# g8a9/multi-modal-emotion

Hardware: AMD Instinct MI355X
Metric: utterances/sec fwd+bwd (+clip_grad_norm_+AdamW inside the timed step), TAV (BERT+Wav2Vec2+VideoMAE) b=32, 1/2/4/8 MI355X (higher is better)
Workload: dtype bf16; 1 GPU; tav_nn.py TAV preset B (bert 12 L + wav2vec2 12 L / 768 + videomae 12 L / 768 on 16 frames + fusion 12 L), global batch 32 = 32 per GPU x 1, text 128 tok, audio 80000 samples, video 16x3x224x224 (104 fusion / 1464 encoder tokens), 547.0 GFLOP forward per utterance; global_batch=32, per_gpu_batch=32, parallelism=dp1, weights=random init (seeded), no checkpoints offline, launch=hipGraph replay

## Files before the change

include/tavhip.h:

```cpp
#ifndef TAVHIP_H
#define TAVHIP_H
#include <stdint.h>

#ifdef __cplusplus
extern "C" {
#endif

enum { TAV_F32 = 0, TAV_BF16 = 1, TAV_FP8 = 2 ,
       TAV_U8 = 3 ,
       TAV_I16 = 4  };
enum {
    TAV_ERR_NULL = -1,
    TAV_ERR_SHAPE = -2,
    TAV_ERR_DTYPE = -3,
    TAV_ERR_ALIGN = -4,
    TAV_ERR_NO_RCCL = -5
};

int tav_version(void);
const char* tav_error_string(int code);

typedef struct tav_gemm_nt_args {
    const void* A; const void* B; void* C;
    void* C_pre;
    const float* bias;
    const void* gelu_in;
    const float* resid;
    int64_t M, N, K;
    int64_t lda, ldb, ldc, ld_pre, ld_gelu_in, ld_resid;
    int32_t nzb, nzg;
    int64_t a_zb, a_zg, b_zb, b_zg, c_zb, c_zg, bias_zg;
    int32_t in_dtype, out_dtype;
    int32_t act;
    int32_t accumulate;
    float alpha;
    const float* a_dequant;
    const float* b_dequant;
    int64_t gelu_zb;
    int32_t tile_m_hint;
} tav_gemm_nt_args;
int tav_gemm_nt(const tav_gemm_nt_args* args, void* stream);
int tav_gemm_nt_schedule(const tav_gemm_nt_args* args, int32_t* tile, int32_t* rows_first, int32_t* tile_rest);

typedef struct tav_gemm_tn_args {
    const void* A; const void* B;
    float* slabs;
    float* out;
    float* dbias;
    float* bias_partials;
    int64_t N1, N2;
    int64_t lda, ldb;
    int64_t rows_per_batch, nbatch;
    int64_t a_zb, b_zb;
    int32_t chunk_rows, nsplit;
    int32_t perm_inner, perm_outer;
    int32_t dtype;
    int32_t accumulate;
    float scale;
} tav_gemm_tn_args;
int tav_gemm_tn_splits(int64_t n1, int64_t n2, int64_t rows_per_batch, int64_t nbatch, int32_t* chunk_rows, int32_t* nsplit);
int tav_gemm_tn(const tav_gemm_tn_args* args, void* stream);

typedef struct tav_gemm_tn_problem {
    const void* A; const void* B;
    float* out;
    float* dbias;
    int64_t N1, N2, lda, ldb;
} tav_gemm_tn_problem;
int tav_gemm_tn_grouped(const tav_gemm_tn_problem* problems, int32_t nproblems, int64_t rows, int32_t dtype, void* stream);
int64_t tav_gemm_tn_grouped_ws_bytes(const tav_gemm_tn_problem* problems, int32_t nproblems, int64_t rows, int32_t dtype, int32_t flags);
int tav_gemm_tn_grouped_ws(const tav_gemm_tn_problem* problems, int32_t nproblems, int64_t rows, int32_t dtype, void* workspace,
                           int64_t workspace_bytes, int32_t flags, void* stream);

int tav_fp8_amax_partials(int64_t rows, int64_t cols);
int tav_fp8_amax(const void* x, int32_t dtype, int64_t rows, int64_t cols, int64_t ld, float* partials, float* scales, void* stream);
int tav_fp8_quantize(const void* x, int32_t dtype, int64_t rows, int64_t cols, int64_t ld, const float* scales, void* q, int64_t ld_q, void* qt,
                     int64_t ld_qt, int64_t rows_pad, void* stream);
int tav_fp8_quantize_delayed(const void* x, int32_t dtype, int64_t rows, int64_t cols, int64_t ld, float* state, void* q, int64_t ld_q, void* qt,
                             int64_t ld_qt, int64_t rows_pad, void* stream);
int tav_fp8_roll_states(float* states, int64_t n, void* stream);
int tav_splitk_reduce(const float* slabs, float* out, int32_t nsplit, int64_t n_elems, int32_t accumulate, void* stream);

int tav_colsum(const void* x, int32_t dtype, int64_t M, int64_t N, int64_t ld, float* partials, int32_t nparts, float* out,
               int32_t accumulate, void* stream);

typedef struct tav_attn_args {
    const void* q; const void* k; const void* v;
    void* o;
    const float* key_mask;
    float* lse;
    float* corr;
    void* o_soft;
    const void* dout; void* dq; void* dk; void* dv;
    float* delta;
    int64_t B, S, nheads;
    int64_t ld_q, ld_k, ld_v, ld_o, ld_do, ld_dq, ld_dk, ld_dv;
    int32_t dtype, mask_mode;
    float scale;
    int32_t q_prescaled;
} tav_attn_args;
int tav_attn_fwd(const tav_attn_args* args, void* stream);
int tav_attn_bwd(const tav_attn_args* args, void* stream);
int tav_attn_fwd_len(const tav_attn_args* args, const int32_t* seq_lens, void* stream);
int tav_attn_bwd_len(const tav_attn_args* args, const int32_t* seq_lens, void* stream);
int tav_attn_probs(const tav_attn_args* args, float* probs, const float* head_scale, int64_t hs_bstride, void* stream);
int tav_head_scale(const void* a, const void* b, void* out, int32_t dtype, const float* head_scale, int64_t hs_bstride, float c0, int64_t B, int64_t S,
                   int64_t nheads, int64_t lda, int64_t ldb, int64_t ldo, void* stream);

typedef struct tav_ln_args {
    const void* x; int32_t x_dtype;
    const float* gamma; const float* beta;
    float* y_f32; void* y_lp; int32_t lp_dtype;
    float* mean; float* rstd;
    const void* dy; int32_t dy_dtype;
    const float* dx_add;
    float* dx_f32; void* dx_lp;
    float* dgamma; float* dbeta; float* partials; int32_t accumulate_params;
    int64_t rows, W;
    int64_t ld_x, ld_y, ld_dy, ld_dx;
    float eps;
    int32_t act;
    int32_t defer_param_reduce;
} tav_ln_args;
// ... 172 lines not shown
```

multi-modal-emotion_amd/csrc/gemm_plan.h:

```cpp
#pragma once
#include <stdint.h>
#include <algorithm>
#include "../../include/tavhip.h"

namespace tav {
namespace plan {

inline int elem_size(int dtype) { return dtype == TAV_FP8 ? 1 : (dtype == TAV_BF16 ? 2 : 4); }

inline int nt_validate(const tav_gemm_nt_args* a, bool need_ptrs) {
    if (!a || (need_ptrs && (!a->A || !a->B || !a->C))) return TAV_ERR_NULL;
    if (a->M <= 0 || a->N <= 0 || a->K <= 0) return TAV_ERR_SHAPE;
    const int es = elem_size(a->in_dtype);
    if (a->in_dtype != TAV_BF16 && a->in_dtype != TAV_F32 && a->in_dtype != TAV_FP8) return TAV_ERR_DTYPE;
    if (a->in_dtype == TAV_F32 && a->out_dtype != TAV_F32) return TAV_ERR_DTYPE;
    if (a->out_dtype != TAV_F32 && a->out_dtype != TAV_BF16) return TAV_ERR_DTYPE;
    if ((a->K * es) % 128 != 0) return TAV_ERR_SHAPE;
    if ((a->M * a->lda + a->K) * es >= (1ll << 32) || (a->N * a->ldb + a->K) * es >= (1ll << 32)) return TAV_ERR_SHAPE;
    if (a->N % 4 != 0) return TAV_ERR_SHAPE;
    {
        const int64_t ldmax = std::max(std::max(a->ldc, a->C_pre ? a->ld_pre : 0), std::max(a->gelu_in ? a->ld_gelu_in : 0, a->resid ? a->ld_resid : 0));
        if (ldmax < 0 || 256 * ldmax + a->N >= (1ll << 30)) return TAV_ERR_SHAPE;
    }
    const int pk = 16 / es;
    if (a->lda % pk || a->ldb % pk || a->ldc % 4) return TAV_ERR_ALIGN;
    if (a->a_zb % pk || a->a_zg % pk || a->b_zb % pk || a->b_zg % pk || a->c_zb % 4 || a->c_zg % 4 || a->gelu_zb % 4) return TAV_ERR_ALIGN;
    return 0;
}

inline int nt_small_tile(int M, int N, int nz) {
    const int tiles_n = (N + 127) / 128;
    int tm = 4;
    double best = 1e30;
    for (int c = 4; c >= 2; --c) {
        const long tiles = (long)((M + 32 * c - 1) / (32 * c)) * tiles_n * nz;
        const double cost = (double)((tiles + 255) / 256) * (c + 0.8);
        if (cost < best - 1e-9) { best = cost; tm = c; }
    }
    return tm;
}
inline double nt_small_us(int M, int N, double nk, int nz, int tm, int epi) {
    static const double slots[5] = {0, 0, 768, 512, 512}, tk[5] = {0, 0, 0.56, 0.72, 0.85}, fix[5] = {0, 0, 3.6, 4.0, 4.4};
    const long t = (long)((M + 32 * tm - 1) / (32 * tm)) * ((N + 127) / 128) * nz;
    const double e = ((epi & 1) ? 2.0 + 0.2 * nk : 0.0) + ((epi & 2) ? 2.0 : 0.0) + ((epi & 4) ? 2.0 : 0.0) + ((epi & 8) ? 1.0 : 0.0) + ((epi & 16) ? 2.5 : 0.0);
    const double kt = (nk <= 36.0 ? nk : 36.0 + 1.6 * (nk - 36.0)) * tk[tm];
    return (double)((long)((t + slots[tm] - 1) / slots[tm])) * (kt + fix[tm] + e * tm / 4.0);
}
inline double nt_big_round_us(double nk, int epi) {
    const double kt = nk * 1.45;
    return kt + 6.5 + ((epi & 1) ? 9.0 : 0.0) + ((epi & 2) ? 4.0 : 0.0) + ((epi & 4) ? 3.0 : 0.0) + ((epi & 8) ? 4.7 : 0.0) + ((epi & 16) ? 6.7 : 0.0);
}
inline int nt_pick_tile(int M, int N, int K, int nz, bool bf16_in, int epi, int* rows_big = nullptr, int* tm_rest = nullptr) {
    int tm = nt_small_tile(M, N, nz);
    if (rows_big) *rows_big = M;
    if (bf16_in && M >= 256 && N >= 256) {
        const double nk = (double)K / 64.0;
        const long tn_big = (N + 255) / 256;
        const long t_big = (long)((M + 255) / 256) * tn_big * nz;
        const double us_small = nt_small_us(M, N, nk, nz, tm, epi);
        const double big_round = nt_big_round_us(nk, epi);
        const double us_big = (double)((t_big + 255) / 256) * big_round;
        double us_best = us_small;
        if (us_big < 0.98 * us_small) { tm = 16; us_best = us_big; }
        const long full = t_big / 256;
        if (rows_big && nz == 1 && full >= 1 && t_big % 256 != 0) {
            const long m_tiles = full * 256 / tn_big;
            const int rows_a = (int)(m_tiles * 256), m_rest = M - rows_a;
            if (m_tiles >= 1 && m_rest > 0) {
                const int tr = nt_small_tile(m_rest, N, 1);
                const double us_split = (double)((m_tiles * tn_big + 255) / 256) * big_round + nt_small_us(m_rest, N, nk, 1, tr, epi) + 2.0;
                if (us_split < 0.93 * us_best) { tm = 16; *rows_big = rows_a; *tm_rest = tr; }
            }
        }
    }
    return tm;
}
inline void nt_plan(const tav_gemm_nt_args* a, int* tm_out, int* rows_big, int* tm_rest) {
    const int es = elem_size(a->in_dtype);
    const int nz = (int)((a->nzb > 0 ? a->nzb : 1) * (a->nzg > 0 ? a->nzg : 1));
    int tm = a->tile_m_hint & 31;
    const bool may_split = tm == 0 && a->in_dtype == TAV_BF16 && nz == 1;
    *rows_big = (int)a->M; *tm_rest = 4;
    if (a->in_dtype == TAV_F32 && (tm == 8 || tm == 16)) tm = 4;
    if (tm != 8 && tm != 16 && (tm < 2 || tm > 4))
        tm = nt_pick_tile((int)a->M, (int)a->N, (int)(a->K * es / 2), nz, a->in_dtype != TAV_F32,
                          ((a->resid || a->accumulate) ? 1 : 0) | (a->out_dtype == TAV_F32 ? 2 : 0) | ((a->act & 3) ? 4 : 0) | (a->gelu_in ? 8 : 0) | (a->C_pre ? 16 : 0),
                          may_split ? rows_big : nullptr, tm_rest);
    if (a->in_dtype == TAV_FP8 && tm != 16) tm = 4;
    *tm_out = tm;
}

enum { EPI_GEN = 0, EPI_PLAIN = 1, EPI_RESID = 2, EPI_GELU_D = 3, EPI_MUL_D = 4 };

#define TAV_NT_TILES(X, IN, OUT, NST, EPI) X(IN, OUT, 4, NST, 4, 4, EPI) X(IN, OUT, 3, NST, 4, 4, EPI) X(IN, OUT, 2, NST, 4, 4, EPI)
#define TAV_NT_FLAVOUR(X, IN, OUT, EPI) X(IN, OUT, 4, 2, 8, 8, EPI) TAV_NT_TILES(X, IN, OUT, 4, EPI) TAV_NT_TILES(X, IN, OUT, 2, EPI)
#define TAV_NT_FLAVOUR3(X, IN, OUT, EPI) \
    X(IN, OUT, 4, 2, 8, 8, EPI) X(IN, OUT, 4, 3, 8, 4, GEN) TAV_NT_TILES(X, IN, OUT, 4, EPI) TAV_NT_TILES(X, IN, OUT, 3, GEN) TAV_NT_TILES(X, IN, OUT, 2, EPI)
#define TAV_NT_KERNELS(X)                                                                                                        \
                                  \
    X(FP8, BF16, 4, 2, 8, 8, PLAIN) X(FP8, BF16, 4, 2, 8, 8, GELU_D) X(FP8, BF16, 4, 2, 8, 8, MUL_D) X(FP8, BF16, 4, 2, 8, 8, GEN) \
    X(FP8, F32, 4, 2, 8, 8, PLAIN) X(FP8, F32, 4, 2, 8, 8, RESID) X(FP8, F32, 4, 2, 8, 8, GEN)                                    \
    X(FP8, BF16, 4, 2, 4, 4, GEN) X(FP8, F32, 4, 2, 4, 4, GEN)                                                                    \
    TAV_NT_FLAVOUR3(X, BF16, BF16, PLAIN) TAV_NT_FLAVOUR(X, BF16, BF16, GELU_D) TAV_NT_FLAVOUR(X, BF16, BF16, MUL_D) TAV_NT_FLAVOUR(X, BF16, BF16, GEN) \
    TAV_NT_FLAVOUR3(X, BF16, F32, PLAIN) TAV_NT_FLAVOUR(X, BF16, F32, RESID) TAV_NT_FLAVOUR(X, BF16, F32, GEN)                    \
                                                                               \
    X(F32, F32, 4, 2, 4, 4, GEN) X(F32, F32, 3, 2, 4, 4, GEN) X(F32, F32, 2, 2, 4, 4, GEN)

struct NtKey {
    int8_t in, out, tm, nst, nw, tnw, epi;
};
constexpr bool operator==(const NtKey& a, const NtKey& b) {
    return a.in == b.in && a.out == b.out && a.tm == b.tm && a.nst == b.nst && a.nw == b.nw && a.tnw == b.tnw && a.epi == b.epi;
}
#define TAV_NT_KEY(IN, OUT, TM, NST, NW, TNW, EPI) {TAV_##IN, TAV_##OUT, TM, NST, NW, TNW, EPI_##EPI},
constexpr NtKey nt_keys[] = {TAV_NT_KERNELS(TAV_NT_KEY)};
#undef TAV_NT_KEY
constexpr int nt_num_keys = (int)(sizeof(nt_keys) / sizeof(nt_keys[0]));
inline int nt_key_index(const NtKey& k) {
    for (int i = 0; i < nt_num_keys; ++i)
        if (nt_keys[i] == k) return i;
    return -1;
}

struct NtLaunch {
    NtKey key;
    int tiles_m, tiles_n;
    unsigned grid_x, grid_y, block;
    size_t lds;
};
inline NtLaunch nt_launch(const tav_gemm_nt_args* a, int M, int tm) {
    const int in = a->in_dtype, out = a->out_dtype;
    const int nzb = a->nzb > 0 ? a->nzb : 1, nzg = a->nzg > 0 ? a->nzg : 1;
    const int bm = tm >= 8 ? 256 : 32 * tm, bn = tm == 16 ? 256 : 128;
    NtLaunch L;
    L.tiles_m = (M + bm - 1) / bm;
    L.tiles_n = ((int)a->N + bn - 1) / bn;
    const long wgs = (long)L.tiles_m * L.tiles_n * nzb * nzg;
    int nst = (a->tile_m_hint >> 5) & 7;
    if (tm == 8) nst = 3;
    else if (tm == 16) nst = 2;
    else if (nst < 2 || nst > 4) nst = (wgs <= 256 && in == TAV_BF16) ? 4 : 2;
    if (in != TAV_BF16) nst = 2;
    L.grid_x = (unsigned)(L.tiles_m * L.tiles_n); L.grid_y = (unsigned)(nzb * nzg); L.block = tm >= 8 ? 512 : 256;
    L.lds = (tm == 16 && in == TAV_BF16) ? (size_t)160 * 1024 : (size_t)nst * (bm + bn) * 128;
    const bool side = a->resid || a->C_pre || a->gelu_in || a->accumulate;
    int epi = EPI_GEN;
    if (!side && a->act == 0) epi = EPI_PLAIN;
    else if (a->resid && !a->C_pre && !a->gelu_in && !a->accumulate && a->act == 0 && out == TAV_F32) epi = EPI_RESID;
    else if (a->C_pre && (a->act & 3) == 3 && !a->resid && !a->gelu_in && !a->accumulate && out == TAV_BF16) epi = EPI_GELU_D;
    else if (a->gelu_in && (a->act & 4) && !(a->act & 3) && !a->resid && !a->C_pre && !a->accumulate && out == TAV_BF16) epi = EPI_MUL_D;
    if (nst == 3 || in == TAV_F32 || (in == TAV_FP8 && tm != 16)) epi = EPI_GEN;
    L.key = NtKey{(int8_t)in, (int8_t)out, (int8_t)(tm >= 8 ? 4 : tm), (int8_t)nst, (int8_t)(tm >= 8 ? 8 : 4), (int8_t)(tm == 16 ? 8 : 4), (int8_t)epi};
    return L;
}

struct NtSplit {
    int M_rest;
    long a_bytes, c_bytes, pre_bytes, gelu_bytes, resid_elems;
};
inline NtSplit nt_split(const tav_gemm_nt_args* a, int rows_big) {
    const long r = rows_big, es = elem_size(a->in_dtype), oes = elem_size(a->out_dtype);
    return NtSplit{(int)a->M - rows_big, r * a->lda * es, r * a->ldc * oes, r * a->ld_pre * oes, r * a->ld_gelu_in * es, r * a->ld_resid};
}

constexpr int TN_PROBLEMS_MAX = 4;

inline int tn_validate_problem(const void* A, const void* B, const void* out, int64_t N1, int64_t N2, int64_t lda, int64_t ldb, int64_t a_zb,
                               int64_t b_zb, int64_t rows_per_batch, int64_t nbatch, int dtype) {
    if (!A || !B || !out) return TAV_ERR_NULL;
    if (N1 <= 0 || N2 <= 0 || rows_per_batch <= 0 || nbatch <= 0) return TAV_ERR_SHAPE;
    if (dtype != TAV_BF16 && dtype != TAV_F32) return TAV_ERR_DTYPE;
    const int es = elem_size(dtype), pk = 16 / es;
    if (N1 % pk || N2 % pk || N2 % 4) return TAV_ERR_SHAPE;
    if (lda % pk || ldb % pk || a_zb % pk || b_zb % pk) return TAV_ERR_ALIGN;
    if ((rows_per_batch + 64) * (lda > ldb ? lda : ldb) * es >= (1ll << 32)) return TAV_ERR_SHAPE;
    return 0;
}
inline int tn_validate_group(const tav_gemm_tn_problem* probs, int nprob, int64_t rows, int dtype) {
    for (int k = 0; k < nprob; ++k) {
        const tav_gemm_tn_problem& a = probs[k];
        const int rc = tn_validate_problem(a.A, a.B, a.out, a.N1, a.N2, a.lda, a.ldb, 0, 0, rows, 1, dtype);
        if (rc != 0) return rc;
    }
    return 0;
}

constexpr double TN_SPLIT_PENALTY = 0.06;
inline void tn_splits(int64_t n1, int64_t n2, int64_t rows_per_batch, int64_t nbatch, int32_t* chunk_rows, int32_t* nsplit) {
    const long tiles = ((n1 + 127) / 128) * ((n2 + 127) / 128);
    const long SLOTS = 512;
    long best_cpb = 1, best_cr = ((rows_per_batch + 63) / 64) * 64; double best_score = -1.0;
    const long max_cpb = (rows_per_batch + 255) / 256 > 0 ? (rows_per_batch + 255) / 256 : 1;
    for (long cpb = 1; cpb <= max_cpb && cpb <= 64; ++cpb) {
        long cr = (rows_per_batch + cpb - 1) / cpb;
        cr = ((cr + 63) / 64) * 64;
        const long real_cpb = (rows_per_batch + cr - 1) / cr;
        const long wgs = tiles * real_cpb * nbatch;
        const long rounds = (wgs + SLOTS - 1) / SLOTS;
        const double work = (double)rounds * (double)cr;
        const double ideal = (double)tiles * nbatch * rows_per_batch / SLOTS;
        const double score = ideal / work - TN_SPLIT_PENALTY * (double)(real_cpb * nbatch);
        if (score > best_score + 1e-9) { best_score = score; best_cpb = real_cpb; best_cr = cr; }
    }
    *chunk_rows = (int32_t)best_cr;
    *nsplit = (int32_t)(best_cpb * nbatch);
}

struct TnGroupPlan {
    bool big;
    int tw, nsplit;
    long chunk;
    long ws_floats;
};
inline TnGroupPlan tn_big_plan(const tav_gemm_tn_problem* probs, int nprob, long rows, int dtype, int flags) {
    TnGroupPlan P{false, 128, 1, 0, 0};
    const bool can_big = dtype == TAV_BF16 && !(flags & 2);
    long tiles = 0, elems = 0;
    for (int k = 0; k < nprob; ++k) {
        tiles += ((probs[k].N1 + 255) / 256) * ((probs[k].N2 + 255) / 256);
        elems += probs[k].N1 * probs[k].N2;
    }
    P.big = can_big && ((flags & 1) || (rows >= 12288 && tiles >= 48));
    if (P.big) {
        int best = 1; double best_score = -1.0;
        for (int s2 = 1; s2 <= 4; ++s2) {
            if (s2 > 1 && rows / s2 < 2048) break;
            const long wgs = tiles * s2;
            const double fill = (double)wgs / (double)(((wgs + 255) / 256) * 256);
            const double score = fill - 0.04 * (s2 - 1);
            if (score > best_score + 1e-9) { best_score = score; best = s2; }
        }
        if ((flags >> 8) & 15) best = (flags >> 8) & 15;
        P.nsplit = best;
        P.tw = 256;
    }
// ... 50 lines not shown
```

multi-modal-emotion_amd/engine.py:

```python
import weakref

import torch

from . import ops

_EPOCH = [0]


def bump_weight_epoch():
    _EPOCH[0] += 1


class Policy:

    def __init__(self, name="bf16", fp8_fwd=None, fp8_bwd=None):
        name = {"bfloat16": "bf16", "float32": "fp32", "f32": "fp32", "float8": "fp8", "e4m3": "fp8"}.get(name, name)
        if name not in ("bf16", "fp32", "fp8", "fp8-all", "fp8-wgrad8"):
            raise ValueError(f"unknown precision policy {name!r}")
        self.name = name
        self.lp = torch.float32 if name == "fp32" else torch.bfloat16
        self.f32 = name == "fp32"
        self.fp8 = name.startswith("fp8")
        self.fp8_stacks = () if not self.fp8 else (("video", "text", "audio", "fusion") if name == "fp8-all" else ("video",))
        self.fp8_wgrad8 = name in ("fp8-wgrad8", "fp8-all")
# ... 177 lines not shown
def _to_lp(pol, x32):
    return x32 if pol.f32 else ops.cast2d(x32, pol.lp)


_LP_HINT = {}


def _hint_set(g32, glp):
    if glp is not None and g32 is not None and g32.is_cuda:
        _LP_HINT[torch.cuda.current_stream().cuda_stream] = (g32, glp)


def _hint_take(g):
    if not g.is_cuda:
        return None
    e = _LP_HINT.pop(torch.cuda.current_stream().cuda_stream, None)
    return e[1] if e is not None and e[0] is g else None


def _c(t):
    return t if t is None or t.is_contiguous() else t.contiguous()


class LayerSpec:
    def __init__(self, B, S, nheads, eps, pre_ln, mask_mode=0, branch=None, head_scale=None, probs_out=None, seq_lens=None):
        self.B, self.S, self.nheads, self.eps, self.pre_ln, self.mask_mode, self.branch = B, S, nheads, eps, pre_ln, mask_mode, branch
        self.seq_lens = seq_lens
        self.head_scale, self.probs_out = head_scale, probs_out


QSC = ops.ATTN_Q_PRESCALE


def _layer_wgrads(pairs, into=None):
    tiles = sum(((a.shape[1] + 127) // 128) * ((b.shape[1] + 127) // 128) for a, b in pairs)
    if len(pairs) <= 4 and tiles >= 256:
        return ops.gemm_tn_grouped(pairs, want_bias=True, into=into)
    return [ops.gemm_tn(a, b, want_bias=True) for a, b in pairs]


def _arena_into(wq, wk, wv, bq, bk, bv, wo, bo, w1, b1, w2, b2):
    from . import runtime as _rt
    if not _rt.grad_slots:
        return None
    g = lambda p: _rt.grad_slots.pop(p.data_ptr(), None) if p is not None else None

    def fused(ps):
        if any(p is None for p in ps):
            return None
        v = _rt.fused_slot(ps)
        for p in ps:
            _rt.grad_slots.pop(p.data_ptr(), None)
        return v
    return [(g(w2), g(b2)), (g(w1), g(b1)), (g(wo), g(bo)), (fused((wq, wk, wv)), fused((bq, bk, bv)))]


def _fp8_layer(pol, spec):
    return bool(pol.fp8 and spec.branch in pol.fp8_stacks)


def _fp8_sites(ectx, spec, wq):
    pol, fp8 = ectx.pol, _fp8_layer(ectx.pol, spec)
    st = lambda tag: ectx.cache.fp8_state(wq, tag)
    return (True, pol.fp8_fwd, pol.fp8_bwd, pol.fp8_wgrad8, st) if fp8 else (False, 0, 0, False, st)


class EncoderLayerFn(torch.autograd.Function):

    @staticmethod
    def forward(ctx, x, x_lp, key_mask, ectx, spec, *params):
        pol, cache = ectx.pol, ectx.cache
        (ln1_w, ln1_b, wq, bq, wk, bk, wv, bv, wo, bo, ln2_w, ln2_b, w1, b1, w2, b2) = params
        B, S, nh = spec.B, spec.S, spec.nheads
        H = nh * 64
        fp8, fm, _, w8, st = _fp8_sites(ectx, spec, wq)
        if not fp8:
            from . import runtime as _rt
            _rt.note_layer_group(wq, wk, wv, bq, bk, bv, wo, bo, w1, b1, w2, b2)
        wqkv, _, bqkv, wo_n, _, w1_n, _, w2_n, _ = cache.layer(wq, wk, wv, bq, bk, bv, wo, w1, w2, q_scale=QSC)
        wqkv8, _, wo8, w18, w28 = cache.layer_fp8(wq, wk, wv, bq, bk, bv, wo, w1, w2, q_scale=QSC) if fp8 else (None,) * 5

        def lin(bit, inp, w_n, w_8, tag, **kw):
            if not fm & bit:
                return ops.gemm_nt(inp, w_n, **kw), None
            inp8 = ops.fp8_quantize(inp, want_t=w8, state=st(tag))
            return ops.gemm_nt_fp8(inp8, w_8, **kw), inp8

        x = _c(x)
        if spec.pre_ln:
            _, a, mean1, rstd1 = _ln_fwd(pol, x, ln1_w, ln1_b, spec.eps, need_f32=False)
        else:
            a = x_lp if x_lp is not None else _to_lp(pol, x)
            mean1 = rstd1 = None
        qkv, a8 = lin(1, a, wqkv, wqkv8, "a", bias=bqkv)
        o, lse, aux = ops.attn_fwd(qkv[:, :H], qkv[:, H:2 * H], qkv[:, 2 * H:], B, S, nh, key_mask=key_mask, mask_mode=spec.mask_mode, q_prescaled=True,
                                   seq_lens=spec.seq_lens)
        hs, o_ctx = spec.head_scale, o
        if hs is not None:
            if spec.mask_mode == 2:
                o_ctx = ops.head_scale(o, aux[1], hs, -1.0, B, S, nh)
            elif spec.mask_mode == 0:
                o_ctx = ops.head_scale(None, o, hs, 0.0, B, S, nh)
            else:
                raise NotImplementedError("head_mask with a pre-softmax key mask is not on any path of the reference")
        if spec.probs_out is not None:
            spec.probs_out.append(ops.attn_probs(qkv[:, :H], qkv[:, H:2 * H], lse, B, S, nh, key_mask=key_mask, mask_mode=spec.mask_mode,
                                                 q_prescaled=True, head_scale=hs))
        y1, o8 = lin(2, o_ctx, wo_n, wo8, "o", bias=bo, resid=x, out_dtype=torch.float32)
        if spec.pre_ln:
            x1 = y1
            _, c, mean2, rstd2 = _ln_fwd(pol, x1, ln2_w, ln2_b, spec.eps, need_f32=False)
        else:
            x1, c, mean1, rstd1 = _ln_fwd(pol, y1, ln1_w, ln1_b, spec.eps, need_f32=True)
        (h, u), c8 = lin(4, c, w1_n, w18, "c", bias=b1, act=3, want_pre=True)
        y2, h8 = lin(8, h, w2_n, w28, "h", bias=b2, resid=x1, out_dtype=torch.float32)
        if spec.pre_ln:
            x2, x2_lp = y2, None
        else:
            x2, x2_lp, mean2, rstd2 = _ln_fwd(pol, y2, ln2_w, ln2_b, spec.eps, need_f32=True)
        ctx.ectx, ctx.spec = ectx, spec
        ctx.set_materialize_grads(False)
        ctx.has = [p is not None for p in params]
        corr, o_soft = aux
        if w8:
            a = c = h = None
            keep8 = tuple(t for x8 in (a8, o8, c8, h8) for t in (x8.qt, x8.scales))
        else:
            keep8 = (None,) * 8
        ctx.save_for_backward(x if spec.pre_ln else None, a, qkv, o, lse, corr, o_soft, y1, c, u, h, y2 if not spec.pre_ln else None,
                              mean1, rstd1, mean2, rstd2, key_mask, o_ctx if hs is not None else None, hs, *keep8, *params)
        if x2_lp is None or pol.f32:
            x2_lp = x2.new_empty(0)
        ctx.mark_non_differentiable(x2_lp)
        return x2, x2_lp

    @staticmethod
    def backward(ctx, g2, _g_lp):
        pol, cache, spec = ctx.ectx.pol, ctx.ectx.cache, ctx.spec
        sv = ctx.saved_tensors
        x, a, qkv, o, lse, corr, o_soft, y1, c, u, h, y2, mean1, rstd1, mean2, rstd2, key_mask, o_ctx, hs = sv[:19]
        (ln1_w, ln1_b, wq, bq, wk, bk, wv, bv, wo, bo, ln2_w, ln2_b, w1, b1, w2, b2) = sv[27:]
        B, S, nh = spec.B, spec.S, spec.nheads
        H, M = nh * 64, qkv.shape[0]
        fp8, _, bm, w8, st = _fp8_sites(ctx.ectx, spec, wq)
        _, wqkv_t, _, _, wo_t, _, w1_t, _, w2_t = cache.layer(wq, wk, wv, bq, bk, bv, wo, w1, w2, q_scale=QSC)
        _, wqkv8, wo8, w18, w28 = cache.layer_fp8(wq, wk, wv, bq, bk, bv, wo, w1, w2, q_scale=QSC) if fp8 else (None,) * 5
        if w8:
            a8, o8, c8, h8 = (ops.Fp8(None, t, s, M, t.shape[0]) for t, s in zip(sv[19:27:2], sv[20:27:2]))
        dgrad_out = pol.lp if pol.dgrad_lp and not fp8 else torch.float32

        def dgrad(dy_lp, bit, w_8, w_t, **kw):
            if bm & bit:
                dy8 = ops.fp8_quantize(dy_lp, want_t=w8, state=st(f"dY{bit}"))
                return ops.gemm_nt(dy8.q, w_8.qt[:, :w_8.rows], a_dequant=dy8.dequant, b_dequant=w_8.dequant, **kw), dy8
            return ops.gemm_nt(dy_lp, w_t, **kw), None

        g2 = _c(g2)
        if spec.pre_ln:
            hint = None if pol.f32 else _hint_take(g2)
            dy2, dy2_lp = g2, (hint if hint is not None else _to_lp(pol, g2))
            dg2 = db2 = None
        else:
            dy2, dy2_lp, dg2, db2 = _ln_bwd(pol, g2, y2, ln2_w, ln2_b, mean2, rstd2)
        du, dy28 = dgrad(dy2_lp, 8, w28, w2_t, gelu_in=u, act=4)
        if spec.pre_ln:
            dc, du8 = dgrad(du, 4, w18, w1_t, out_dtype=dgrad_out)
            g1, g1_lp, dg2, db2 = _ln_bwd(pol, dc, y1, ln2_w, ln2_b, mean2, rstd2, dx_add=dy2)
            dy1, dy1_lp = g1, g1_lp
        else:
            g1, du8 = dgrad(du, 4, w18, w1_t, resid=dy2, out_dtype=torch.float32)
            dy1, dy1_lp, dg1, db1 = _ln_bwd(pol, g1, y1, ln1_w, ln1_b, mean1, rstd1)
        do, dy18 = dgrad(dy1_lp, 2, wo8, wo_t)
        qs, ks, vs = qkv[:, :H], qkv[:, H:2 * H], qkv[:, 2 * H:]
        if hs is None:
            dqkv = ops.attn_bwd(qs, ks, vs, o, do, lse, (corr, o_soft) if spec.mask_mode == 2 else None,
                                B, S, nh, key_mask=key_mask, mask_mode=spec.mask_mode, q_prescaled=True, seq_lens=spec.seq_lens)
        elif spec.mask_mode == 2:
            dqkv = ops.attn_bwd(qs, ks, vs, o, do, lse, (corr, o_soft), B, S, nh, key_mask=key_mask, mask_mode=2, q_prescaled=True)
            dqkv2 = ops.attn_bwd(qs, ks, vs, o_soft, ops.head_scale(None, do, hs, -1.0, B, S, nh), lse, None, B, S, nh, mask_mode=0, q_prescaled=True)
            ops.head_scale(dqkv, dqkv2, None, 1.0, B, S, 3 * nh, out=dqkv)
        else:
            dqkv = ops.attn_bwd(qs, ks, vs, o, ops.head_scale(None, do, hs, 0.0, B, S, nh), lse, None, B, S, nh, mask_mode=0, q_prescaled=True)
        if hs is not None:
            o = o_ctx
        if spec.pre_ln:
            da, dqkv8 = dgrad(dqkv, 1, wqkv8, wqkv_t, out_dtype=dgrad_out)
            g0, g0_lp, dg1, db1 = _ln_bwd(pol, da, x, ln1_w, ln1_b, mean1, rstd1, dx_add=dy1, need_lp=not pol.f32)
            if not pol.f32:
                _hint_set(g0, g0_lp)
        else:
            g0, dqkv8 = dgrad(dqkv, 1, wqkv8, wqkv_t, resid=dy1, out_dtype=torch.float32)
        if w8:
            dW2, dW1, dWo, dWqkv = ops.wgrad_fp8(dy28, h8), ops.wgrad_fp8(du8, c8), ops.wgrad_fp8(dy18, o8), ops.wgrad_fp8(dqkv8, a8)
            dB2, dB1, dBo, dBqkv = ops.colsum(dy2_lp), ops.colsum(du), ops.colsum(dy1_lp), ops.colsum(dqkv)
        else:
            into = None if fp8 else _arena_into(wq, wk, wv, bq, bk, bv, wo, bo, w1, b1, w2, b2)
            (dW2, dB2), (dW1, dB1), (dWo, dBo), (dWqkv, dBqkv) = _layer_wgrads([(dy2_lp, h), (du, c), (dy1_lp, o), (dqkv, a)], into)
        grads = [dg1, db1, dWqkv[:H], dBqkv[:H], dWqkv[H:2 * H], dBqkv[H:2 * H], dWqkv[2 * H:], dBqkv[2 * H:], dWo, dBo, dg2, db2, dW1, dB1, dW2, dB2]
        grads = [g if has else None for g, has in zip(grads, ctx.has)]
        return (g0, None, None, None, None, *grads)


def encoder_layer(ectx, spec, x, x_lp, key_mask, params):
    fp8, slow = _fp8_layer(ectx.pol, spec), spec.head_scale is not None or spec.probs_out is not None
    if fp8 and slow:
        raise NotImplementedError("head_mask / output_attentions are built for the bf16 and fp32 policies only")
    if fp8 and spec.seq_lens is not None:
        raise ValueError("per-row sequence lengths (seq_lens) are built for the bf16 and fp32 policies only, not fp8")
    if slow and spec.seq_lens is not None:
        raise NotImplementedError("head_mask / output_attentions are not built for per-row sequence lengths (seq_lens)")
    x2, x2_lp = EncoderLayerFn.apply(x, x_lp, key_mask, ectx, spec, *params)
    return x2, (x2_lp if x2_lp.numel() else None)


class LinearFn(torch.autograd.Function):

    @staticmethod
    def forward(ctx, x32, x_lp, w, b, resid, ectx, out_f32):
        pol = ectx.pol
        if x_lp is None:
            x_lp = _to_lp(pol, _c(x32))
        w_n, _ = ectx.cache.linear(w)
        y = ops.gemm_nt(x_lp, w_n, bias=b, resid=resid, out_dtype=torch.float32 if out_f32 else pol.lp)
        ctx.ectx = ectx
        ctx.in_f32 = x32 is not None
        ctx.save_for_backward(x_lp, w, b)
        return y

    @staticmethod
    def backward(ctx, gy):
        pol = ctx.ectx.pol
        x_lp, w, b = ctx.saved_tensors
        _, w_t = ctx.ectx.cache.linear(w)
        gy = _c(gy)
        gy_lp = gy if gy.dtype == pol.lp else _to_lp(pol, gy)
        dW = dB = None
        if ctx.needs_input_grad[2]:
            if b is not None and ctx.needs_input_grad[3]:
# ... 690 lines not shown
```

multi-modal-emotion_amd/ops.py:

```python
import collections
import ctypes as C
import math

import numpy as np
import torch

from . import _lib as L
from ._lib import check, dt, lib, ptr, stream

_ws = {}


def workspace(name, nfloats, device):
    key = (name, torch.cuda.current_stream().cuda_stream, str(device))
    t = _ws.get(key)
    if t is None or t.numel() < nfloats:
        t = torch.empty(max(int(nfloats), 1), dtype=torch.float32, device=device)
        _ws[key] = t
    return t


def clear_workspaces():
    _ws.clear()


_prof = None


def profile_start(kinds):
    global _prof
    _prof = {"kinds": {kinds} if isinstance(kinds, str) else set(kinds), "ev": []}


def _prof_launch(family, select, work, nbytes, launch, work_exec=None):
    if _prof is not None and family in _prof["kinds"]:
        e0, e1 = torch.cuda.Event(enable_timing=True), torch.cuda.Event(enable_timing=True)
        e0.record()
        launch()
        e1.record()
        _prof["ev"].append((e0, e1, float(work), select, float(nbytes), family, float(work if work_exec is None else work_exec)))
    else:
        launch()


def profile_stop(select="bf16"):
    global _prof
    torch.cuda.synchronize()
    allev, _prof = _prof["ev"], None
    fam = {}
    for e0, e1, work, sel, nbytes, family, work_exec in allev:
        d = fam.setdefault(family, {"work": 0.0, "work_exec": 0.0, "bytes": 0.0, "secs": 0.0, "launches": 0})
        d["work"] += work
        d["work_exec"] += work_exec
        d["bytes"] += nbytes
        d["secs"] += e0.elapsed_time(e1) * 1e-3
        d["launches"] += 1
    profile_stop.families = fam
    ev = [e for e in allev if e[5] == "gemm_nt" and e[3] == select]
    secs = sum(e[0].elapsed_time(e[1]) for e in ev) * 1e-3
    profile_stop.algorithmic_bytes = sum(e[4] for e in ev)
    return sum(e[2] for e in ev), secs, len(ev)


def gemm_nt(a, b, *, bias=None, act=0, resid=None, gelu_in=None, out_dtype=None, want_pre=False, out=None,
            accumulate=False, alpha=1.0, M=None, N=None, K=None, lda=None, ldb=None, ldc=None,
            nzb=1, nzg=1, a_zb=0, a_zg=0, b_zb=0, b_zg=0, c_zb=0, c_zg=0, bias_zg=0, out_shape=None, tile_m=0, a_dequant=None, b_dequant=None,
            ld_gelu=None, gelu_zb=0):
    if M is None:
        M, K = a.shape[-2], a.shape[-1]
        N = b.shape[-2]
        lda, ldb = a.stride(-2), b.stride(-2)
    out_dtype = out_dtype or (torch.bfloat16 if a.dtype == torch.float8_e4m3fn else a.dtype)
    if out is None:
        out = torch.empty(out_shape or (M, N), dtype=out_dtype, device=a.device)
    if ldc is None:
        ldc = out.stride(-2)
    pre = torch.empty_strided(out.shape, out.stride(), dtype=out.dtype, device=out.device) if want_pre else None
    g = L.GemmNTArgs()
    g.A, g.B, g.C, g.C_pre = ptr(a), ptr(b), ptr(out), ptr(pre)
    g.bias, g.gelu_in, g.resid = ptr(bias), ptr(gelu_in), ptr(resid)
    g.M, g.N, g.K = M, N, K
    g.lda, g.ldb, g.ldc, g.ld_pre = lda, ldb, ldc, ldc
    g.ld_gelu_in = (ld_gelu if ld_gelu is not None else gelu_in.stride(-2)) if gelu_in is not None else 0
    g.gelu_zb = gelu_zb
    g.ld_resid = resid.stride(-2) if resid is not None else 0
    g.nzb, g.nzg = nzb, nzg
    g.a_zb, g.a_zg, g.b_zb, g.b_zg, g.c_zb, g.c_zg, g.bias_zg = a_zb, a_zg, b_zb, b_zg, c_zb, c_zg, bias_zg
    g.in_dtype, g.out_dtype, g.act, g.accumulate, g.alpha = dt(a), dt(out), act, int(accumulate), alpha
    g.tile_m_hint = tile_m
    g.a_dequant, g.b_dequant = ptr(a_dequant), ptr(b_dequant)
    if bias is not None:
        assert bias.dtype == torch.float32
    if resid is not None:
        assert resid.dtype == torch.float32
    if gelu_in is not None:
        assert gelu_in.dtype == (torch.bfloat16 if a.dtype == torch.float8_e4m3fn else a.dtype)
    nz = max(nzb, 1) * max(nzg, 1)
    osz = 4 if out_dtype == torch.float32 else 2
    nbytes = nz * ((M * K + N * K) * a.element_size() + M * N * (osz * (2 if want_pre else 1) + (4 if resid is not None else 0)
                                                                 + (2 if gelu_in is not None else 0) + (osz if accumulate else 0)))
    sel = "bf16" if a.dtype == torch.bfloat16 else ("fp8" if a.dtype == torch.float8_e4m3fn else "f32")
    _prof_launch("gemm_nt", sel, 2.0 * M * N * K * nz, nbytes, lambda: check(lib().tav_gemm_nt(C.byref(g), stream()), "gemm_nt"))
    return (out, pre) if want_pre else out


def gemm_tn(a, b, *, out=None, accumulate=False, N1=None, N2=None, lda=None, ldb=None, rows_per_batch=None, nbatch=1,
            a_zb=0, b_zb=0, perm_inner=0, perm_outer=0, scale=1.0, out_shape=None, want_bias=False):
    if N1 is None:
        N1, N2 = a.shape[-1], b.shape[-1]
        rows_per_batch = a.shape[-2]
        lda, ldb = a.stride(-2), b.stride(-2)
    cr, ns = C.c_int32(), C.c_int32()
    check(lib().tav_gemm_tn_splits(N1, N2, rows_per_batch, nbatch, C.byref(cr), C.byref(ns)), "gemm_tn_splits")
    slabs = workspace("tn_slabs", ns.value * N1 * N2, a.device)
    if out is None:
        out = torch.empty(out_shape or (N1, N2), dtype=torch.float32, device=a.device)
    g = L.GemmTNArgs()
    g.A, g.B, g.slabs, g.out = ptr(a), ptr(b), ptr(slabs), ptr(out)
    g.N1, g.N2, g.lda, g.ldb = N1, N2, lda, ldb
    g.rows_per_batch, g.nbatch, g.a_zb, g.b_zb = rows_per_batch, nbatch, a_zb, b_zb
    g.chunk_rows, g.nsplit, g.perm_inner, g.perm_outer = cr.value, ns.value, perm_inner, perm_outer
    g.dtype, g.accumulate, g.scale = dt(a), int(accumulate), scale
    dbias = None
    if want_bias:
        dbias = torch.empty(N1, dtype=torch.float32, device=a.device)
        bpart = workspace("tn_bias", ns.value * N1, a.device)
        g.dbias, g.bias_partials = ptr(dbias), ptr(bpart)
    assert a.dtype == b.dtype
    tokens = rows_per_batch * nbatch
    _prof_launch("gemm_tn", "bf16" if a.dtype == torch.bfloat16 else "f32", 2.0 * tokens * N1 * N2, tokens * (N1 + N2) * a.element_size() + 4 * N1 * N2,
                 lambda: check(lib().tav_gemm_tn(C.byref(g), stream()), "gemm_tn"))
    return (out, dbias) if want_bias else out


def gemm_tn_grouped(pairs, want_bias=True, flags=0, into=None):
    n = len(pairs)
    rows, dtype = pairs[0][0].shape[0], pairs[0][0].dtype
    probs = (L.GemmTNProblem * n)()
    outs = []
    for k, (a, b) in enumerate(pairs):
        assert a.shape[0] == rows and b.shape[0] == rows and a.dtype == dtype and b.dtype == dtype
        N1, N2 = a.shape[1], b.shape[1]
        dW_to, db_to = into[k] if into is not None else (None, None)
        dW = dW_to if dW_to is not None else torch.empty(N1, N2, dtype=torch.float32, device=a.device)
# ... 1187 lines not shown
```

Baseline: 437.5 utterances/s.

## Add 192x256 BF16 GEMM tile variant and opt-in planner hint for encoder linears

Adds a new 192-row by 256-column macro-tile configuration for BF16 NT GEMMs, with its own cost model in the tile planner. The new tile is enabled through a hint bit that the encoder linear and dgrad calls now pass. It is picked only when the whole grid fits in one wave of 256 workgroups and the model predicts it beats the existing choice, aiming to cut wave-quantization tail waste. It also fixes the split-path bookkeeping so the best estimate is updated, and adds seven new kernel instantiations that raise compile time and binary size.

Measured after the change: 435.8 utterances/s. About the same (-0.4%).

```diff
diff --git a/include/tavhip.h b/include/tavhip.h
--- a/include/tavhip.h
+++ b/include/tavhip.h
@@ -39,6 +39,7 @@
     int64_t gelu_zb;
     int32_t tile_m_hint;
 } tav_gemm_nt_args;
+#define TAV_NT_HINT_192 256
 int tav_gemm_nt(const tav_gemm_nt_args* args, void* stream);
 int tav_gemm_nt_schedule(const tav_gemm_nt_args* args, int32_t* tile, int32_t* rows_first, int32_t* tile_rest);
 
diff --git a/multi-modal-emotion_amd/csrc/gemm_plan.h b/multi-modal-emotion_amd/csrc/gemm_plan.h
--- a/multi-modal-emotion_amd/csrc/gemm_plan.h
+++ b/multi-modal-emotion_amd/csrc/gemm_plan.h
@@ -6,6 +6,7 @@
 namespace tav {
 namespace plan {
 
+constexpr int NT_HINT_192 = TAV_NT_HINT_192;
 inline int elem_size(int dtype) { return dtype == TAV_FP8 ? 1 : (dtype == TAV_BF16 ? 2 : 4); }
 
 inline int nt_validate(const tav_gemm_nt_args* a, bool need_ptrs) {
@@ -50,7 +51,11 @@
     const double kt = nk * 1.45;
     return kt + 6.5 + ((epi & 1) ? 9.0 : 0.0) + ((epi & 2) ? 4.0 : 0.0) + ((epi & 4) ? 3.0 : 0.0) + ((epi & 8) ? 4.7 : 0.0) + ((epi & 16) ? 6.7 : 0.0);
 }
-inline int nt_pick_tile(int M, int N, int K, int nz, bool bf16_in, int epi, int* rows_big = nullptr, int* tm_rest = nullptr) {
+inline double nt_192_round_us(double nk, int epi) {
+    const double kt = nk * 1.07;
+    return kt + 9.25 + ((epi & 1) ? 5.35 : 0.0) + ((epi & 2) ? 2.05 : 0.0) + ((epi & 4) ? 1.4 : 0.0) + ((epi & 8) ? 1.15 : 0.0) + ((epi & 16) ? 3.15 : 0.0);
+}
+inline int nt_pick_tile(int M, int N, int K, int nz, bool bf16_in, int epi, int* rows_big = nullptr, int* tm_rest = nullptr, bool opt192 = false) {
     int tm = nt_small_tile(M, N, nz);
     if (rows_big) *rows_big = M;
     if (bf16_in && M >= 256 && N >= 256) {
@@ -69,8 +74,12 @@
             if (m_tiles >= 1 && m_rest > 0) {
                 const int tr = nt_small_tile(m_rest, N, 1);
                 const double us_split = (double)((m_tiles * tn_big + 255) / 256) * big_round + nt_small_us(m_rest, N, nk, 1, tr, epi) + 2.0;
-                if (us_split < 0.93 * us_best) { tm = 16; *rows_big = rows_a; *tm_rest = tr; }
+                if (us_split < 0.93 * us_best) { tm = 16; *rows_big = rows_a; *tm_rest = tr; us_best = us_split; }
             }
+        }
+        if (opt192 && nz == 1) {
+            const long t_192 = (long)((M + 191) / 192) * tn_big;
+            if (t_192 <= 256 && nt_192_round_us(nk, epi) < 0.93 * us_best) { tm = 12; if (rows_big) *rows_big = M; }
         }
     }
     return tm;
@@ -79,13 +88,16 @@
     const int es = elem_size(a->in_dtype);
     const int nz = (int)((a->nzb > 0 ? a->nzb : 1) * (a->nzg > 0 ? a->nzg : 1));
     int tm = a->tile_m_hint & 31;
+    const bool opt192 = (a->tile_m_hint & NT_HINT_192) != 0 && a->in_dtype == TAV_BF16;
+    const bool force192 = tm == 12 && a->in_dtype == TAV_BF16;
     const bool may_split = tm == 0 && a->in_dtype == TAV_BF16 && nz == 1;
     *rows_big = (int)a->M; *tm_rest = 4;
     if (a->in_dtype == TAV_F32 && (tm == 8 || tm == 16)) tm = 4;
-    if (tm != 8 && tm != 16 && (tm < 2 || tm > 4))
+    if (force192) tm = opt192 ? 12 : 16;
+    else if (tm != 8 && tm != 16 && (tm < 2 || tm > 4))
         tm = nt_pick_tile((int)a->M, (int)a->N, (int)(a->K * es / 2), nz, a->in_dtype != TAV_F32,
                           ((a->resid || a->accumulate) ? 1 : 0) | (a->out_dtype == TAV_F32 ? 2 : 0) | ((a->act & 3) ? 4 : 0) | (a->gelu_in ? 8 : 0) | (a->C_pre ? 16 : 0),
-                          may_split ? rows_big : nullptr, tm_rest);
+                          may_split ? rows_big : nullptr, tm_rest, opt192);
     if (a->in_dtype == TAV_FP8 && tm != 16) tm = 4;
     *tm_out = tm;
 }
@@ -104,7 +116,10 @@
     TAV_NT_FLAVOUR3(X, BF16, BF16, PLAIN) TAV_NT_FLAVOUR(X, BF16, BF16, GELU_D) TAV_NT_FLAVOUR(X, BF16, BF16, MUL_D) TAV_NT_FLAVOUR(X, BF16, BF16, GEN) \
     TAV_NT_FLAVOUR3(X, BF16, F32, PLAIN) TAV_NT_FLAVOUR(X, BF16, F32, RESID) TAV_NT_FLAVOUR(X, BF16, F32, GEN)                    \
                                                                                \
-    X(F32, F32, 4, 2, 4, 4, GEN) X(F32, F32, 3, 2, 4, 4, GEN) X(F32, F32, 2, 2, 4, 4, GEN)
+    X(F32, F32, 4, 2, 4, 4, GEN) X(F32, F32, 3, 2, 4, 4, GEN) X(F32, F32, 2, 2, 4, 4, GEN)                                        \
+     \
+    X(BF16, BF16, 3, 2, 8, 8, PLAIN) X(BF16, BF16, 3, 2, 8, 8, GELU_D) X(BF16, BF16, 3, 2, 8, 8, MUL_D) X(BF16, BF16, 3, 2, 8, 8, GEN) \
+    X(BF16, F32, 3, 2, 8, 8, PLAIN) X(BF16, F32, 3, 2, 8, 8, RESID) X(BF16, F32, 3, 2, 8, 8, GEN)
 
 struct NtKey {
     int8_t in, out, tm, nst, nw, tnw, epi;
@@ -131,18 +146,19 @@
 inline NtLaunch nt_launch(const tav_gemm_nt_args* a, int M, int tm) {
     const int in = a->in_dtype, out = a->out_dtype;
     const int nzb = a->nzb > 0 ? a->nzb : 1, nzg = a->nzg > 0 ? a->nzg : 1;
-    const int bm = tm >= 8 ? 256 : 32 * tm, bn = tm == 16 ? 256 : 128;
+    const bool t192 = in == TAV_BF16 && (tm == 12 || (tm == 16 && (a->tile_m_hint & 31) == 12));
+    const int bm = t192 ? 192 : (tm >= 8 ? 256 : 32 * tm), bn = (tm == 16 || t192) ? 256 : 128;
     NtLaunch L;
     L.tiles_m = (M + bm - 1) / bm;
     L.tiles_n = ((int)a->N + bn - 1) / bn;
     const long wgs = (long)L.tiles_m * L.tiles_n * nzb * nzg;
     int nst = (a->tile_m_hint >> 5) & 7;
     if (tm == 8) nst = 3;
-    else if (tm == 16) nst = 2;
+    else if (tm == 16 || t192) nst = 2;
     else if (nst < 2 || nst > 4) nst = (wgs <= 256 && in == TAV_BF16) ? 4 : 2;
     if (in != TAV_BF16) nst = 2;
     L.grid_x = (unsigned)(L.tiles_m * L.tiles_n); L.grid_y = (unsigned)(nzb * nzg); L.block = tm >= 8 ? 512 : 256;
-    L.lds = (tm == 16 && in == TAV_BF16) ? (size_t)160 * 1024 : (size_t)nst * (bm + bn) * 128;
+    L.lds = t192 ? (size_t)136 * 1024 : (tm == 16 && in == TAV_BF16) ? (size_t)160 * 1024 : (size_t)nst * (bm + bn) * 128;
     const bool side = a->resid || a->C_pre || a->gelu_in || a->accumulate;
     int epi = EPI_GEN;
     if (!side && a->act == 0) epi = EPI_PLAIN;
@@ -150,7 +166,7 @@
     else if (a->C_pre && (a->act & 3) == 3 && !a->resid && !a->gelu_in && !a->accumulate && out == TAV_BF16) epi = EPI_GELU_D;
     else if (a->gelu_in && (a->act & 4) && !(a->act & 3) && !a->resid && !a->C_pre && !a->accumulate && out == TAV_BF16) epi = EPI_MUL_D;
     if (nst == 3 || in == TAV_F32 || (in == TAV_FP8 && tm != 16)) epi = EPI_GEN;
-    L.key = NtKey{(int8_t)in, (int8_t)out, (int8_t)(tm >= 8 ? 4 : tm), (int8_t)nst, (int8_t)(tm >= 8 ? 8 : 4), (int8_t)(tm == 16 ? 8 : 4), (int8_t)epi};
+    L.key = NtKey{(int8_t)in, (int8_t)out, (int8_t)(t192 ? 3 : tm >= 8 ? 4 : tm), (int8_t)nst, (int8_t)(tm >= 8 ? 8 : 4), (int8_t)((tm == 16 || t192) ? 8 : 4), (int8_t)epi};
     return L;
 }
 
diff --git a/multi-modal-emotion_amd/engine.py b/multi-modal-emotion_amd/engine.py
--- a/multi-modal-emotion_amd/engine.py
+++ b/multi-modal-emotion_amd/engine.py
@@ -283,7 +283,7 @@
 
         def lin(bit, inp, w_n, w_8, tag, **kw):
             if not fm & bit:
-                return ops.gemm_nt(inp, w_n, **kw), None
+                return ops.gemm_nt(inp, w_n, tile_m=ops.NT_HINT_192, **kw), None
             inp8 = ops.fp8_quantize(inp, want_t=w8, state=st(tag))
             return ops.gemm_nt_fp8(inp8, w_8, **kw), inp8
 
@@ -354,7 +354,7 @@
             if bm & bit:
                 dy8 = ops.fp8_quantize(dy_lp, want_t=w8, state=st(f"dY{bit}"))
                 return ops.gemm_nt(dy8.q, w_8.qt[:, :w_8.rows], a_dequant=dy8.dequant, b_dequant=w_8.dequant, **kw), dy8
-            return ops.gemm_nt(dy_lp, w_t, **kw), None
+            return ops.gemm_nt(dy_lp, w_t, tile_m=ops.NT_HINT_192, **kw), None
 
         g2 = _c(g2)
         if spec.pre_ln:
diff --git a/multi-modal-emotion_amd/ops.py b/multi-modal-emotion_amd/ops.py
--- a/multi-modal-emotion_amd/ops.py
+++ b/multi-modal-emotion_amd/ops.py
@@ -60,6 +60,9 @@
     secs = sum(e[0].elapsed_time(e[1]) for e in ev) * 1e-3
     profile_stop.algorithmic_bytes = sum(e[4] for e in ev)
     return sum(e[2] for e in ev), secs, len(ev)
+
+
+NT_HINT_192 = 256
 
 
 def gemm_nt(a, b, *, bias=None, act=0, resid=None, gelu_in=None, out_dtype=None, want_pre=False, out=None,
```
